# AntonXue/nn-sdp

Measured on NVIDIA B200. Metric: queries/sec (clique LMI blocks assembled: value * cliques_per_query), higher is better.
Workload: dtype f64

## Files before the change

include/nnsdp_b200.h:

```cpp
#ifndef NNSDP_B200_H
#define NNSDP_B200_H

#include <stdint.h>

#ifdef __cplusplus
extern "C" {
#endif

#define NNSDP_OK 0
#define NNSDP_ERR_ARG (-1)
#define NNSDP_ERR_CUDA (-2)
#define NNSDP_ERR_NOMEM (-3)
#define NNSDP_ERR_STATE (-4)
#define NNSDP_ERR_ASSERT (-5)
#define NNSDP_ERR_NOCONV (-6)

#define NNSDP_OUT_SAFETY 0
#define NNSDP_OUT_HPLANE 1
#define NNSDP_OUT_CIRCLE 2
#define NNSDP_OUT_ELLIPSOID 3

#define NNSDP_FORMAT_BLOCKS 0
#define NNSDP_FORMAT_DENSE_Z 1
#define NNSDP_FORMAT_PACKED 2
// ... 60 lines not shown
int32_t nnsdp_cliques(const nnsdp_net* net, int64_t beta, int64_t* ck_off, int64_t* ck_idx,
                      int64_t* ck1_len, int64_t* d_off, int64_t* d_idx);
int32_t nnsdp_sizes_from_xdims(int64_t K, const int64_t* xdims, int64_t beta, nnsdp_sizes* sizes);
int32_t nnsdp_cliques_from_xdims(int64_t K, const int64_t* xdims, int64_t beta, int64_t* ck_off,
                                 int64_t* ck_idx, int64_t* ck1_len, int64_t* d_off, int64_t* d_idx);

int32_t nnsdp_plan_stats(int64_t K, const int64_t* xdims, int64_t beta, int32_t dense_Z,
                         int64_t* tiles_per_prog, int64_t* entries_per_prog, int64_t* tile_rows,
                         int64_t* tile_cols);

int32_t nnsdp_plan_tiles(int64_t K, const int64_t* xdims, int64_t beta, int32_t dense_Z,
                         int64_t max_tiles, int32_t* tiles_out, int64_t* ntiles);

int32_t nnsdp_plan_panel(int64_t K, const int64_t* xdims, int64_t beta, int32_t dense_Z, int64_t max_items,
                         int64_t* items_out, int64_t* nitems);

int32_t nnsdp_gather_plan(int64_t K, const int64_t* xdims, int64_t beta, int32_t dense_Z, int64_t max_cells,
                          int32_t* cells_out, int64_t* ncells, int64_t max_thin, int64_t* thin_out,
                          int64_t* nthin, int32_t* usable);

int32_t nnsdp_bounds_ibp(nnsdp_ctx* ctx, const nnsdp_net* net, int64_t Q, const double* x1min,
                         const double* x1max, double* xmin, double* xmax, double* acxmin,
                         double* acxmax);
int32_t nnsdp_bounds_crown(nnsdp_ctx* ctx, const nnsdp_net* net, int64_t Q, const double* x1min,
                           const double* x1max, double* xmin, double* xmax, double* acxmin, double* acxmax);
int32_t nnsdp_preact_from_x(nnsdp_ctx* ctx, const nnsdp_net* net, int64_t Q, const double* xmin,
                            const double* xmax, double* acxmin, double* acxmax);
int32_t nnsdp_sector_minmax(nnsdp_ctx* ctx, int64_t n, const double* acxmin, const double* acxmax,
                            double* smin, double* smax);
int32_t nnsdp_assemble_blocks(nnsdp_ctx* ctx, const nnsdp_net* net, int64_t beta, int64_t Q,
// ... 110 lines not shown
```

nn-sdp_b200/csrc/api.cu:

```cuda
#include <math.h>
#include <stdarg.h>
#include <stdio.h>
#include <stdlib.h>
#include <string.h>

#include <algorithm>
#include <cmath>
#include <condition_variable>
#include <deque>
#include <functional>
#include <memory>
#include <mutex>
#include <thread>
#include <unordered_map>

#include <cuda.h>

#include "internal.h"

namespace nnsdp {

static thread_local std::string g_err;

void set_error(const char* fmt, ...) {
// ... 207 lines not shown
  DevBuf xmin, xmax, acxmin, acxmax, smin_c, smax_c;
  DevBuf d11, Md, T0, Bt, u, aff, part, act, cnt, Z11, Z1K, U;
  DevBuf gram, ringbuf, flags;
  DevBuf cr_rowsA, cr_rowsB, cr_bias, cr_prel, cr_preu, cr_du, cr_bu, cr_dl;
  DevBuf cr_keep_l, cr_keep_u;
  bool keep_preact = false, preact_valid = false;
  BatchDev bd{};
  GramDev gd{};
  PlanDev pd{};
  bool have_inputs = false, bounds_supplied = false, bounds_done = false, prepared = false;
  bool shared_gram = false;
  int bounds_method = 0;
  cudaStream_t st = nullptr, st_copy = nullptr;
  cudaEvent_t ev_start = nullptr, ev_stop = nullptr;
  cudaEvent_t ev_done[2] = {nullptr, nullptr}, ev_free[2] = {nullptr, nullptr};
  std::vector<StageSpan> spans;
  std::vector<cudaEvent_t> ev_pool;
  float stage_ms[ST_COUNT] = {};
  int64_t stage_launches[ST_COUNT] = {};

  cudaEvent_t get_event() {
    if (!ev_pool.empty()) {
      cudaEvent_t e = ev_pool.back();
      ev_pool.pop_back();
      return e;
    }
    cudaEvent_t e = nullptr;
    cudaEventCreate(&e);
    return e;
  }
// ... 15 lines not shown
    for (auto& sp : spans) {
      float ms = 0.f;
      if (cudaEventElapsedTime(&ms, sp.e0, sp.e1) == cudaSuccess) {
        stage_ms[sp.stage] += ms;
        if (sp.stage >= 5 && sp.stage <= 7) stage_ms[3] += ms;
      }
      ev_pool.push_back(sp.e0);
      ev_pool.push_back(sp.e1);
    }
    spans.clear();
  }
  std::vector<DevBuf*> all_bufs() {
    return {&d_bands, &d_tmaps, &d_tmap_ok, &d_tiles, &d_strips, &d_bulk, &d_mats, &d_panel, &d_goff, &d_ldG, &d_chol, &ze_netv, &ze_g, &ze_rows, &ze_part, &ze_io, &ze_err, &x1min, &x1max, &ymin, &ymax, &smin, &smax,
            &gin, &gbnd, &gsec, &outS, &outvec, &outinvP, &gout, &xmin, &xmax, &acxmin, &acxmax,
            &smin_c, &smax_c, &d11, &Md, &T0, &Bt, &u, &aff, &part, &act, &cnt, &Z11, &Z1K, &U,
            &gram, &ringbuf, &flags, &cr_rowsA, &cr_rowsB, &cr_bias, &cr_prel, &cr_preu, &cr_du, &cr_bu, &cr_dl,
            &cr_keep_l, &cr_keep_u};
  }
};

namespace {

int32_t require_device() {
  int n = 0;
  cudaError_t e = cudaGetDeviceCount(&n);
  if (e != cudaSuccess || n <= 0) {
    cudaGetLastError();
    set_error("no CUDA device available (%s); this library has no CPU fallback",
              e == cudaSuccess ? "device count is 0" : cudaGetErrorString(e));
    return NNSDP_ERR_CUDA;
  }
// ... 325 lines not shown
  Shape sh;
  NN_TRY(shape_from_xdims(K, xdims, &sh));
  nnsdp_sizes sz;
  NN_TRY(fill_sizes(sh, beta, &sz));
  std::vector<CliqueRanges> mats;
  NN_TRY(format_mats(sh, beta, dense_Z, &mats));
  PlanHost plan;
  PackedLayout lay;
  NN_TRY(build_plan(sh, beta, mats, true, &plan, dense_Z == NNSDP_FORMAT_PACKED ? &lay : nullptr));
  *ntiles = (int64_t)plan.tiles.size();
  if (tiles_out) {
    NN_CHECK(max_tiles >= *ntiles, NNSDP_ERR_ARG, "tiles_out too small");
    static_assert(sizeof(TileDev) == 11 * sizeof(int32_t), "TileDev layout");
    memcpy(tiles_out, plan.tiles.data(), plan.tiles.size() * sizeof(TileDev));
  }
  return NNSDP_OK;
}

int32_t nnsdp_plan_panel(int64_t K, const int64_t* xdims, int64_t beta, int32_t dense_Z, int64_t max_items,
                         int64_t* items_out, int64_t* nitems) {
  NN_CHECK(nitems != nullptr, NNSDP_ERR_ARG, "NULL argument");
  Shape sh;
  NN_TRY(shape_from_xdims(K, xdims, &sh));
  nnsdp_sizes sz;
  NN_TRY(fill_sizes(sh, beta, &sz));
  std::vector<CliqueRanges> mats;
  NN_TRY(format_mats(sh, beta, dense_Z, &mats));
  PlanHost plan;
  PackedLayout lay;
  NN_TRY(build_plan(sh, beta, mats, true, &plan, dense_Z == NNSDP_FORMAT_PACKED ? &lay : nullptr));
// ... 40 lines not shown
        o[5] = c.kind; o[6] = c.blk; o[7] = c.pure_zero;
      }
  }
  if (thin_out) {
    NN_CHECK(max_thin >= *nthin, NNSDP_ERR_ARG, "thin_out too small");
    memcpy(thin_out, gp.thin_idx.data(), gp.thin_idx.size() * 8);
  }
  return NNSDP_OK;
}

int32_t nnsdp_batch_destroy(nnsdp_batch* b) {
  if (!b) return NNSDP_OK;
  cudaSetDevice(b->dev);
  if (b->st) cudaStreamSynchronize(b->st);
  if (b->st_copy) cudaStreamSynchronize(b->st_copy);
  b->resolve_spans();
  b->pool.reset();
  for (DevBuf* x : b->all_bufs()) x->release();
  b->d_thin_idx.release();
  b->d_packed.release();
  b->d_pairs.release();
  if (b->h_packed) cudaFreeHost(b->h_packed);
  for (cudaEvent_t e : b->ev_packed)
    if (e) cudaEventDestroy(e);
  for (cudaEvent_t e : b->ev_pool) cudaEventDestroy(e);
  for (cudaEvent_t e : {b->ev_start, b->ev_stop, b->ev_done[0], b->ev_done[1], b->ev_free[0], b->ev_free[1]})
    if (e) cudaEventDestroy(e);
  if (b->st) cudaStreamDestroy(b->st);
  if (b->st_copy) cudaStreamDestroy(b->st_copy);
  delete b;
  return NNSDP_OK;
}

int32_t nnsdp_batch_create(nnsdp_ctx* ctx, int32_t dev_index, const nnsdp_net* net, int64_t beta,
                           int64_t Qcap, int64_t ring_queries, int32_t dense_Z, nnsdp_batch** out) {
  NN_CHECK(out != nullptr, NNSDP_ERR_ARG, "batch output pointer is NULL");
  *out = nullptr;
  NN_CHECK(ctx && net, NNSDP_ERR_ARG, "NULL argument");
  NN_CHECK(net->ctx == ctx, NNSDP_ERR_ARG, "net was uploaded through a different ctx");
  NN_CHECK(dev_index >= 0 && dev_index < (int)ctx->devs.size(), NNSDP_ERR_ARG, "bad dev_index");
  NN_CHECK(Qcap >= 1 && Qcap < (1 << 30), NNSDP_ERR_ARG, "bad Qcap");
  NN_CHECK(ring_queries >= 0 && ring_queries <= 65535, NNSDP_ERR_ARG, "ring_queries must be in [0, 65535]");
  const Shape& sh = net->sh;
  nnsdp_batch* b = new nnsdp_batch();
// ... 64 lines not shown
    for (const BandDev& j : b->plan.bands) b->band_max_m = std::max(b->band_max_m, j.m);
    b->nbands = (int)b->plan.bands.size();
    NN_TRY(upload(b->d_bands, b->plan.bands.data(), b->plan.bands.size() * sizeof(BandDev), b->st));
    if (!b->packed) NN_TRY(build_gather_plan(sh, beta, mats, b->plan, &b->gp));
    if (const char* e = getenv("NNSDP_DENSE_GATHER"))
      if (e[0] == '1') b->gp.usable = false;
    if (b->gp.usable) {
      NN_TRY(upload(b->d_thin_idx, b->gp.thin_idx.data(), b->gp.thin_idx.size() * 8, b->st));
      for (int i = 0; i < GATHER_STAGES; ++i)
        NN_CUDA(cudaEventCreateWithFlags(&b->ev_packed[i], cudaEventDisableTiming));
    }
    NN_TRY(upload(b->d_tiles, b->plan.tiles.data(), b->plan.tiles.size() * sizeof(TileDev), b->st));
    NN_TRY(upload(b->d_mats, b->plan.mats.data(), b->plan.mats.size() * sizeof(MatDev), b->st));
    NN_TRY(b->ringbuf.ensure((size_t)b->plan.per_query_doubles * b->ring * 8));
    b->slot_bulk.assign((size_t)b->ring * sh.K, 0);
    auto is_bulk = [&](const StripDev& d) {
      return !b->packed && d.rblk >= 1 && d.rblk <= sh.K - 1 &&
             (d.prog == PROG_SAME || (d.prog == PROG_DIAG && !b->plan.band_inline));
    };
    std::vector<StripDev> strips, bulk;
    std::vector<std::vector<StripDev>> per_blk(sh.K);
    b->pass_entries = 0;
    b->bulk_entries.assign(sh.K, 0);
    for (const StripDev& d : b->plan.strips) {
      if (d.prog == PROG_ZERO) continue;
      if (is_bulk(d)) {
        per_blk[d.rblk].push_back(d);
        b->bulk_entries[d.rblk] += (int64_t)d.nrows * d.ncols;
      } else {
        strips.push_back(d);
        b->pass_entries += (int64_t)d.nrows * d.ncols;
      }
    }
    b->bulk_begin.assign(sh.K + 1, 0);
// ... 4 lines not shown
    b->bulk_begin[sh.K] = (int)bulk.size();
    for (int i = b->plan.n_fill; i < (int)b->plan.tiles.size(); ++i)
      b->pass_entries += (int64_t)b->plan.tiles[i].nrows * b->plan.tiles[i].ncols;
    for (const BandDev& j : b->plan.bands)
      if (j.ld > 0) b->pass_entries += (int64_t)j.m * (2 * beta + 1) - beta * (beta + 1);
    NN_TRY(upload(b->d_strips, strips.data(), strips.size() * sizeof(StripDev), b->st));
    NN_TRY(upload(b->d_bulk, bulk.data(), bulk.size() * sizeof(StripDev), b->st));
    b->pd.strips = b->d_strips.as<StripDev>();
    b->pd.bulk = b->d_bulk.as<StripDev>();
    b->pd.n_strips = (int)strips.size();
    b->pd.tiles = b->d_tiles.as<TileDev>();
    b->pd.mats = b->d_mats.as<MatDev>();
    b->pd.panel_desc = nullptr;
    b->pd.n_panel = 0;
    b->pd.fold = 0;
    {
      static const int panel_env = [] { const char* e = getenv("NNSDP_PANEL"); return e ? atoi(e) : 1; }();
      if (panel_env && !b->packed && !b->plan.panel.empty()) {
        const char* fold_env = getenv("NNSDP_PANEL_FOLD");
        const bool fold = !(fold_env && atoi(fold_env) == 0);
        std::vector<StripDev> panel;
        for (const StripDev& d : fold ? b->plan.panel_fold : b->plan.panel)
          if (d.prog != PROG_ZERO && (d.prog == PROG_RC || d.prog == PROG_CR || !is_bulk(d))) panel.push_back(d);
        NN_TRY(upload(b->d_panel, panel.data(), panel.size() * sizeof(StripDev), b->st));
        b->pd.panel_desc = b->d_panel.as<StripDev>();
        b->pd.n_panel = (int)panel.size();
        b->pd.fold = fold ? 1 : 0;
      }
    }
    b->pd.ntiles = (int)b->plan.tiles.size();
    b->pd.n_fill = b->plan.n_fill;
    b->pd.n_window = b->plan.n_window;
    b->pd.n_edge = b->plan.n_edge;
    b->pd.tile_rows = b->plan.tile_rows;
    b->pd.per_query = b->plan.per_query_doubles;
    b->pd.tmaps = nullptr;
// ... 29 lines not shown
          NN_CUDA(cudaStreamSynchronize(b->st));
          b->pd.tmaps = b->d_tmaps.p;
          b->pd.tmap_ok = b->d_tmap_ok.as<int>();
        }
      } else {
        cudaGetLastError();
      }
    }
    b->pd.packed = b->plan.skip_absent ? 1 : 0;
    b->pd.band_inline = b->plan.band_inline ? 1 : 0;
    b->gd.scratch = b->gram.as<double>();
    b->gd.per_query = go;
    b->gd.goff = b->d_goff.as<long long>();
    b->gd.ldG = b->d_ldG.as<int>();
    b->gd.mirror = b->packed && b->plan.skip_absent ? 0 : 1;
  }
  NN_CUDA(cudaStreamSynchronize(b->st));
  guard.b = nullptr;
  *out = b;
  return NNSDP_OK;
}

int32_t nnsdp_batch_set_inputs(nnsdp_batch* b, int64_t Q, const nnsdp_query_inputs* in) {
  NN_CHECK(b && in, NNSDP_ERR_ARG, "NULL argument");
  NN_CHECK(Q >= 1 && Q <= b->Qcap, NNSDP_ERR_ARG, "Q = %lld outside [1, Qcap = %lld]", (long long)Q,
           (long long)b->Qcap);
  NN_CUDA(cudaSetDevice(b->dev));
  const Shape& sh = b->net->sh;
  const nnsdp_sizes& sz = b->sz;
  BatchDev& bd = b->bd;
// ... 215 lines not shown
    for (int blk = 1; blk < K; ++blk) {
      const int first = b->bulk_begin[blk], count = b->bulk_begin[blk + 1] - first;
      if (count == 0) continue;
      const bool now = blk <= K - 2 ? b->h_cnt[(size_t)q * K + blk] > 0 : b->bd.has_s22 != 0;
      if (now || held[blk]) {
        b->sel.push_back({(int32_t)i, first, count});
        entries += b->bulk_entries[blk];
      }
      held[blk] = now;
    }
  }
  if (!b->packed) b->emitted_bytes += entries * 8;
  return NNSDP_OK;
}

static int32_t emit_pass(nnsdp_batch* b, const GramDev& gd, int q0, int nq, double* dst) {
  const NetPerDev& nd = *b->nd;
  NN_TRY(prepare_slots(b, q0, nq, (dst - b->ringbuf.as<double>()) / b->plan.per_query_doubles));
  int total = 0;
  for (int which = 0; which < 3; ++which) {
    b->span_begin(ST_EMIT_FILL + which, b->st);
    const int l = launch_emit(nd.nd, b->bd, gd, b->pd, q0, nq, dst, b->st, which, b->sel.data(), (int)b->sel.size());
    b->span_end(b->st, l);
    total += l;
  }
  if (b->nbands > 0) {
    b->span_begin(ST_EMIT_EDGE, b->st);
    const int l = launch_emit_band(nd.nd, b->bd, gd, b->d_bands.as<BandDev>(), b->nbands, b->band_max_m, b->pd.per_query,
                                   q0, nq, dst, b->st);
    b->span_end(b->st, l);
    total += l;
  }
  b->stage_launches[ST_EMIT] += total;
  const cudaError_t e = cudaGetLastError();
  if (e != cudaSuccess) {
    b->ring_zeroed = 0;
    return cuda_fail(e, "emitter pass", __FILE__, __LINE__);
  }
  return NNSDP_OK;
}

int32_t nnsdp_batch_emit(nnsdp_batch* b, int64_t q0, int64_t nq) {
  NN_CHECK(b != nullptr, NNSDP_ERR_ARG, "batch is NULL");
  NN_CHECK(b->prepared, NNSDP_ERR_STATE, "nnsdp_batch_emit before nnsdp_batch_prepare");
  NN_CHECK(q0 >= 0 && nq >= 1 && q0 + nq <= b->Q && nq <= b->ring, NNSDP_ERR_ARG,
           "bad query range [%lld, %lld) for Q = %lld, ring = %lld", (long long)q0,
           (long long)(q0 + nq), (long long)b->Q, (long long)b->ring);
// ... 169 lines not shown
    const size_t need = (size_t)GATHER_STAGES * chunk * b->gp.thin_idx.size();
    if (need > b->h_packed_doubles) {
      if (b->h_packed) cudaFreeHost(b->h_packed);
      b->h_packed = nullptr;
      b->h_packed_doubles = 0;
      NN_CUDA(cudaHostAlloc((void**)&b->h_packed, std::max<size_t>(need, 1) * 8, cudaHostAllocPortable));
      b->h_packed_doubles = need;
      NN_TRY(b->d_packed.ensure(std::max<size_t>(need, 1) * 8));
    }
    if (!b->pool) {
      int nt = (int)std::min<unsigned>(16u, std::max(1u, std::thread::hardware_concurrency()));
      if (const char* e = getenv("NNSDP_HOST_THREADS")) nt = std::max(1, atoi(e));
      b->pool.reset(new WorkerPool(nt));
    }
  }
  bool used[2] = {false, false};
  int h = 0, ci = 0;
  int32_t status = NNSDP_OK;
  for (int64_t q0 = 0; q0 < b->Q && status == NNSDP_OK; q0 += chunk, h = (h + 1) % nhalf, ++ci) {
    const int64_t nq = std::min(chunk, b->Q - q0);
    double* dst = b->ringbuf.as<double>() + (int64_t)h * chunk * per;
    GramDev gd = b->gd;
    if (b->shared_gram) gd.per_query = 0;
    else gd.scratch += (int64_t)h * chunk * gd.per_query;
    if (sparse && ci >= GATHER_STAGES) b->pool->wait_group(ci - GATHER_STAGES);
    if (host_out && used[h]) NN_CUDA(cudaStreamWaitEvent(b->st, b->ev_free[h], 0));
    if (!b->shared_gram || ci == 0) {
      b->span_begin(ST_GRAM, b->st);
      int l = b->shared_gram
                  ? launch_gram(nd.nd, b->bd, b->gd, (int)b->net->max_block, 0, b->d_pairs.as<int>(), (int)b->pair_begin[1], b->st)
                  : launch_gram(nd.nd, b->bd, gd, (int)b->net->max_block, (int)q0, b->d_pairs.as<int>() + 2 * b->pair_begin[q0],
                                (int)(b->pair_begin[q0 + nq] - b->pair_begin[q0]), b->st);
      b->span_end(b->st, l > 0 ? l : 0);
      NN_CHECK(l >= 0, NNSDP_ERR_ARG, "a hidden layer of %lld neurons is too wide for the Gram kernel's grid",
               (long long)b->net->max_block);
      NN_CUDA(cudaGetLastError());
    }
    status = emit_pass(b, gd, (int)q0, (int)nq, dst);
    if (status != NNSDP_OK) break;
    if (sparse) {
      status = gather_chunk(b, ci, q0, nq, h, dst, host_out, flags);
      used[h] = true;
    } else if (host_out && b->packed && !(flags & NNSDP_RUN_DENSE_COPY)) {
      NN_CUDA(cudaEventRecord(b->ev_done[h], b->st));
      NN_CUDA(cudaStreamWaitEvent(b->st_copy, b->ev_done[h], 0));
      b->span_begin(ST_D2H, b->st_copy);
      const int64_t alw = b->lay.always_doubles;
      if (alw == per)
        NN_CUDA(cudaMemcpyAsync(host_out + q0 * per, dst, (size_t)nq * per * 8, cudaMemcpyDeviceToHost, b->st_copy));
      else
        NN_CUDA(cudaMemcpy2DAsync(host_out + q0 * per, (size_t)per * 8, dst, (size_t)per * 8, (size_t)alw * 8, (size_t)nq,
                                  cudaMemcpyDeviceToHost, b->st_copy));
      b->gather_bytes_dma += nq * alw * 8;
      for (int64_t q = q0; q < q0 + nq; ++q)
// ... 10 lines not shown
      used[h] = true;
    } else if (host_out) {
      NN_CUDA(cudaEventRecord(b->ev_done[h], b->st));
      NN_CUDA(cudaStreamWaitEvent(b->st_copy, b->ev_done[h], 0));
      b->span_begin(ST_D2H, b->st_copy);
      NN_CUDA(cudaMemcpyAsync(host_out + q0 * per, dst, (size_t)nq * per * 8, cudaMemcpyDeviceToHost,
                              b->st_copy));
      b->span_end(b->st_copy, 0);
      NN_CUDA(cudaEventRecord(b->ev_free[h], b->st_copy));
      used[h] = true;
      b->gather_bytes_dma += nq * per * 8;
    }
  }
  if (b->pool) b->pool->wait_all();
  if (status != NNSDP_OK) {
    cudaStreamSynchronize(b->st);
    cudaStreamSynchronize(b->st_copy);
    return status;
  }
  NN_CUDA(cudaGetLastError());
  NN_CUDA(cudaStreamSynchronize(b->st));
  NN_CUDA(cudaStreamSynchronize(b->st_copy));
  b->resolve_spans();
  return NNSDP_OK;
}

int32_t nnsdp_batch_run_ex(nnsdp_batch* b, double* host_out, int32_t flags) { return run_impl(b, host_out, nullptr, flags); }

int32_t nnsdp_batch_run(nnsdp_batch* b, double* host_out) { return run_impl(b, host_out, nullptr, 0); }

int32_t nnsdp_batch_run_packed(nnsdp_batch* b, double* host_records, uint8_t* present, int32_t flags) {
  NN_CHECK(b != nullptr, NNSDP_ERR_ARG, "batch is NULL");
  NN_CHECK(b->packed, NNSDP_ERR_STATE, "the batch was not created with NNSDP_FORMAT_PACKED");
// ... 1523 lines not shown
```

nn-sdp_b200/csrc/internal.h:

```cpp
#pragma once

#include <cuda_runtime.h>
#include <stdint.h>

#include <string>
#include <vector>

#include "../../include/nnsdp_b200.h"

namespace nnsdp {

void set_error(const char* fmt, ...);
int32_t cuda_fail(cudaError_t e, const char* what, const char* file, int line);

#define NN_CUDA(call)                                                                \
  do {                                                                               \
    cudaError_t _e = (call);                                                         \
    if (_e != cudaSuccess) return ::nnsdp::cuda_fail(_e, #call, __FILE__, __LINE__); \
  } while (0)

#define NN_CHECK(cond, code, ...)      \
  do {                                 \
    if (!(cond)) {                     \
      ::nnsdp::set_error(__VA_ARGS__); \
// ... 136 lines not shown
struct GatherColSeg {
  int32_t mat, col0, ncols;
  std::vector<GatherCell> cells;
};
struct GatherPlan {
  bool usable = false;
  std::vector<GatherColSeg> colsegs;
  std::vector<int32_t> colseg_begin;
  std::vector<int64_t> thin_idx;
  std::vector<int64_t> thin_begin;
  int64_t dense_always_doubles = 0;
};

int32_t build_plan(const Shape& sh, int64_t beta, const std::vector<CliqueRanges>& mats,
                   bool classify, PlanHost* plan, PackedLayout* packed = nullptr);
void unpack_record(const Shape& sh, int64_t beta, const PackedLayout& lay, const std::vector<CliqueRanges>& mats,
                   const double* record, const uint8_t* present, double* out);
int32_t build_gather_plan(const Shape& sh, int64_t beta, const std::vector<CliqueRanges>& mats,
                          const PlanHost& plan, GatherPlan* gp);

struct CholFront {
  long long out_off;
  long long g0;
  int n, npriv;
  int lead, tail;
};
int32_t build_chol_plan(const Shape& sh, const std::vector<CliqueRanges>& mats, std::vector<CholFront>* fronts);

struct NetDev {
  int K, n_in, n_out, Zdim, acdim, xtot;
// ... 204 lines not shown
```

nn-sdp_b200/csrc/kernels_emit.cu:

```cuda
#include <stdlib.h>

#include <algorithm>

#include "internal.h"

namespace nnsdp {

namespace {

constexpr int ETHREADS = 256;
constexpr int SLOT_GROUP = 8;
constexpr int FAST_TR = 128, FAST_TC = 32, FAST_NCOL = 16;
constexpr int MAX_TAPS = 2 * MAX_FAST_BETA + 1;
constexpr int MAX_TC = 32;

struct QView {
  const double* Md;
  const double* T0;
  const double* Bt;
  const double* gbnd;
  const double* aff;
  const double* Z11;
  const double* Z1K;
  const double* U;
// ... 726 lines not shown
    const dim3 grid(plan.n_window * ((nq + wgroup - 1) / wgroup));
    const int t0 = plan.n_fill;
    static const int gm_env = [] { const char* e = getenv("NNSDP_WINDOW_GROUP_MAJOR"); return e ? atoi(e) : -1; }();
    const int gm = gm_env >= 0 ? gm_env : plan.band_inline;
    switch (b.beta) {
      case 0: emit_window_kernel<0><<<grid, ETHREADS, 0, st>>>(net, b, plan, t0, q0, nq, wgroup, gm, out); break;
      case 1: emit_window_kernel<1><<<grid, ETHREADS, 0, st>>>(net, b, plan, t0, q0, nq, wgroup, gm, out); break;
      case 2: emit_window_kernel<2><<<grid, ETHREADS, 0, st>>>(net, b, plan, t0, q0, nq, wgroup, gm, out); break;
      case 3: emit_window_kernel<3><<<grid, ETHREADS, 0, st>>>(net, b, plan, t0, q0, nq, wgroup, gm, out); break;
      case 4: emit_window_kernel<4><<<grid, ETHREADS, 0, st>>>(net, b, plan, t0, q0, nq, wgroup, gm, out); break;
      default: return -1;
    }
    ++launches;
  }
  }
  if (which < 0 || which == 0) launches += launch_bulk(net, b, g, plan, q0, sel, nsel, out, st);
  if (!plan.fold && plan.n_edge > 0 && (which < 0 || which == 2)) {
    emit_edge_kernel<<<dim3(plan.n_edge, (nq + egroup - 1) / egroup), ETHREADS, 0, st>>>(
        net, b, g, plan, plan.n_fill + plan.n_window, q0, nq, egroup, out);
    ++launches;
  }
  return launches;
}

}
```

nn-sdp_b200/csrc/plan.cpp:

```cpp
#include <stdint.h>
#include <stdlib.h>

#include <algorithm>

#include "internal.h"
#include <atomic>
#include <cstring>
#include <thread>

namespace nnsdp {

int64_t lambda_dim(int64_t acdim, int64_t beta) {
  int64_t s = 0;
  for (int64_t t = acdim - beta; t <= acdim; ++t) s += t;
  return s;
}

long long gram_layout(const Shape& sh, std::vector<long long>* goff, std::vector<int>* ldG) {
  goff->assign(sh.K, 0);
  ldG->assign(sh.K, 0);
  long long go = 0;
  for (int blk = 0; blk <= sh.K - 2; ++blk) {
    (*ldG)[blk] = (int)(((sh.n[blk] + 15) / 16) * 16);
    (*goff)[blk] = go;
    go += (long long)(*ldG)[blk] * sh.n[blk];
  }
  return go;
}

static int64_t Sfun(const Shape& sh, int64_t k) {
// ... 848 lines not shown
```

nn-sdp_b200/nnsdp_b200/__init__.py:

```python
from . import _lib
from ._lib import NnsdpError, device_count, OUT_SAFETY, OUT_HPLANE, OUT_CIRCLE, OUT_ELLIPSOID, RUN_HOST_PREZEROED, RUN_DENSE_COPY, FORMAT_BLOCKS, FORMAT_DENSE_Z, FORMAT_PACKED, CELL_WINDOW, CELL_DIAG, CELL_BAND, CELL_RECT
from .core import (Context, Net, Batch, NumericBatch, PinnedBuffer, assemble_blocks, assemble_dense,
                   bounds_ibp, bounds_crown, preact_from_x, sector_minmax, split_blocks, sizes_from_xdims,
                   cliques_from_xdims, plan_stats, plan_tiles, plan_panel, certify_plan, assembly_error_nmax, affine_form, affine_form_batch, gather_plan, read_nnet, read_vnnlib, packed_layout, packed_unpack,
                   assemble_packed)
from . import reference_api
```

nn-sdp_b200/nnsdp_b200/_lib.py:

```python
from __future__ import annotations

import ctypes as C
import os

_HERE = os.path.dirname(os.path.abspath(__file__))
LIB_PATH = os.environ.get("NNSDP_B200_LIB", os.path.join(_HERE, "..", "lib", "libnnsdp_b200.so"))

OK, ERR_ARG, ERR_CUDA, ERR_NOMEM, ERR_STATE, ERR_ASSERT, ERR_NOCONV = 0, -1, -2, -3, -4, -5, -6
OUT_SAFETY, OUT_HPLANE, OUT_CIRCLE, OUT_ELLIPSOID = 0, 1, 2, 3
RUN_HOST_PREZEROED, RUN_DENSE_COPY = 1, 2
FORMAT_BLOCKS, FORMAT_DENSE_Z, FORMAT_PACKED = 0, 1, 2
CELL_WINDOW, CELL_DIAG, CELL_BAND, CELL_RECT = 1, 2, 3, 4

c_i32, c_i64, c_u64 = C.c_int32, C.c_int64, C.c_uint64
c_dp = C.POINTER(C.c_double)
c_i64p = C.POINTER(C.c_int64)
c_vp = C.c_void_p


class Sizes(C.Structure):
    _fields_ = [(n, c_i64) for n in (
        "K", "Zdim", "acdim", "xtot", "lamdim", "secdim", "n_in", "n_out", "sdim", "ncliques",
        "sum_ck", "sum_ck_sq", "sum_dk", "max_ck")]

# ... 48 lines not shown
    "nnsdp_ctx_destroy": (c_i32, [c_vp]),
    "nnsdp_ctx_num_devices": (c_i32, [c_vp, C.POINTER(c_i32)]),
    "nnsdp_host_alloc": (c_i32, [c_u64, C.POINTER(c_vp)]),
    "nnsdp_host_free": (c_i32, [c_vp]),
    "nnsdp_net_upload": (c_i32, [c_vp, c_i64, c_i64p, C.POINTER(c_dp), C.POINTER(c_vp)]),
    "nnsdp_net_destroy": (c_i32, [c_vp]),
    "nnsdp_nnet_read": (c_i32, [C.c_char_p, c_i64, c_i64p, c_i64p, c_i64, c_dp, c_i64p]),
    "nnsdp_vnnlib_read": (c_i32, [C.c_char_p, c_i64, c_i64, c_i64, c_i64p, c_i64p, c_dp, c_dp, c_dp, c_i64p]),
    "nnsdp_query_sizes": (c_i32, [c_vp, c_i64, C.POINTER(Sizes)]),
    "nnsdp_cliques": (c_i32, [c_vp, c_i64, c_i64p, c_i64p, c_i64p, c_i64p, c_i64p]),
    "nnsdp_sizes_from_xdims": (c_i32, [c_i64, c_i64p, c_i64, C.POINTER(Sizes)]),
    "nnsdp_cliques_from_xdims": (c_i32, [c_i64, c_i64p, c_i64, c_i64p, c_i64p, c_i64p, c_i64p, c_i64p]),
    "nnsdp_plan_stats": (c_i32, [c_i64, c_i64p, c_i64, c_i32, c_i64p, c_i64p, c_i64p, c_i64p]),
    "nnsdp_plan_tiles": (c_i32, [c_i64, c_i64p, c_i64, c_i32, c_i64, C.POINTER(c_i32), c_i64p]),
    "nnsdp_plan_panel": (c_i32, [c_i64, c_i64p, c_i64, c_i32, c_i64, c_i64p, c_i64p]),
    "nnsdp_gather_plan": (c_i32, [c_i64, c_i64p, c_i64, c_i32, c_i64, C.POINTER(c_i32), c_i64p, c_i64, c_i64p, c_i64p, C.POINTER(c_i32)]),
    "nnsdp_bounds_ibp": (c_i32, [c_vp, c_vp, c_i64, c_dp, c_dp, c_dp, c_dp, c_dp, c_dp]),
    "nnsdp_bounds_crown": (c_i32, [c_vp, c_vp, c_i64, c_dp, c_dp, c_dp, c_dp, c_dp, c_dp]),
    "nnsdp_batch_bounds_crown": (c_i32, [c_vp]),
    "nnsdp_batch_set_bounds_method": (c_i32, [c_vp, c_i32]),
    "nnsdp_batch_keep_crown_preact": (c_i32, [c_vp, c_i32]),
    "nnsdp_batch_get_crown_preact": (c_i32, [c_vp, c_dp, c_dp]),
    "nnsdp_preact_from_x": (c_i32, [c_vp, c_vp, c_i64, c_dp, c_dp, c_dp, c_dp]),
    "nnsdp_sector_minmax": (c_i32, [c_vp, c_i64, c_dp, c_dp, c_dp, c_dp]),
    "nnsdp_assemble_blocks": (c_i32, [c_vp, c_vp, c_i64, c_i64, C.POINTER(QueryInputs), c_dp]),
    "nnsdp_assemble_dense": (c_i32, [c_vp, c_vp, c_i64, c_i64, C.POINTER(QueryInputs), c_dp]),
    "nnsdp_batch_lambda_max": (c_i32, [c_vp, c_i32, C.c_double, c_dp, C.POINTER(c_i32)]),
    "nnsdp_batch_lambda_max_ex": (c_i32, [c_vp, c_i32, C.c_double, c_dp, C.POINTER(c_i32), c_dp, C.POINTER(c_i32)]),
    "nnsdp_batch_certify": (c_i32, [c_vp, c_dp, c_i64, C.POINTER(c_i32), c_dp, c_i64p, c_dp]),
    "nnsdp_batch_certify_ex": (c_i32, [c_vp, c_dp, c_i64, C.POINTER(c_i32), c_dp, c_i64p, c_dp, c_dp]),
# ... 75 lines not shown
```

nn-sdp_b200/nnsdp_b200/core.py:

```python
from __future__ import annotations

import ctypes as C
from dataclasses import dataclass
from typing import List, Optional, Sequence

import numpy as np

from . import _lib as L

STAGES = {"bounds": 0, "prepare": 1, "gram": 2, "emit": 3, "d2h": 4, "emit_fill": 5, "emit_window": 6, "emit_edge": 7}


def _dp(a: Optional[np.ndarray]):
    return None if a is None else a.ctypes.data_as(L.c_dp)


def _f64(a, shape_tail=None) -> np.ndarray:
    a = np.ascontiguousarray(np.asarray(a, dtype=np.float64))
    return a


class Context:

    def __init__(self, devices=None):
# ... 118 lines not shown
TILE_FIELDS = ("mat", "row0", "nrows", "col0", "ncols", "grow0", "gcol0", "flags", "rblk", "cblk", "prog")


PANEL_FIELDS = ("out_off", "ld", "row0", "nrows", "col0", "ncols", "grow0", "gcol0", "prog", "rblk")


def plan_panel(xdims: Sequence[int], beta: int, dense: int = 0) -> np.ndarray:
    K = len(xdims) - 1
    xd = (L.c_i64 * (K + 1))(*[int(x) for x in xdims])
    n = L.c_i64(0)
    L.check(L.lib.nnsdp_plan_panel(K, xd, beta, int(dense), 0, None, C.byref(n)))
    out = np.zeros((int(n.value), 10), dtype=np.int64)
    if n.value:
        L.check(L.lib.nnsdp_plan_panel(K, xd, beta, int(dense), int(n.value), out.ctypes.data_as(L.c_i64p), C.byref(n)))
    return out


CERTIFY_PLAN_FIELDS = ("out_off", "n", "npriv", "g0", "lead", "tail")


def assembly_error_nmax(xdims: Sequence[int], beta: int, out_kind: int) -> int:
    xd = np.ascontiguousarray(xdims, dtype=np.int64)
    n = L.c_i64(0)
    L.check(L.lib.nnsdp_assembly_error_nmax(len(xd) - 1, xd.ctypes.data_as(L.c_i64p), beta, out_kind, C.byref(n)))
    return int(n.value)


def certify_plan(xdims: Sequence[int], beta: int) -> np.ndarray:
    K = len(xdims) - 1
    xd = (L.c_i64 * (K + 1))(*[int(x) for x in xdims])
# ... 515 lines not shown
```

Measured before the change: 9468.

## Overlap next-chunk Gram and band emission on a side stream

Adds a high-priority side stream that computes the Gram scratch for the next chunk while the current chunk is emitted, using a second Gram buffer and events to ping-pong between them. When a plan-time check shows that band writers do not overlap the other emit writers, the band-edge kernel also runs on the side stream, concurrently with the fill kernels. This is meant to hide Gram and band kernel latency behind the emit work. The cost is extra memory for the second buffer, more event synchronisation, and correctness that depends on the disjointness check.

```diff
diff --git a/include/nnsdp_b200.h b/include/nnsdp_b200.h
--- a/include/nnsdp_b200.h
+++ b/include/nnsdp_b200.h
@@ -98,6 +98,9 @@
 
 int32_t nnsdp_plan_panel(int64_t K, const int64_t* xdims, int64_t beta, int32_t dense_Z, int64_t max_items,
                          int64_t* items_out, int64_t* nitems);
+
+int32_t nnsdp_plan_band_disjoint(int64_t K, const int64_t* xdims, int64_t beta, int32_t dense_Z, const int64_t* items,
+                                 int64_t nitems, int32_t* disjoint);
 
 int32_t nnsdp_gather_plan(int64_t K, const int64_t* xdims, int64_t beta, int32_t dense_Z, int64_t max_cells,
                           int32_t* cells_out, int64_t* ncells, int64_t max_thin, int64_t* thin_out,
diff --git a/nn-sdp_b200/csrc/api.cu b/nn-sdp_b200/csrc/api.cu
--- a/nn-sdp_b200/csrc/api.cu
+++ b/nn-sdp_b200/csrc/api.cu
@@ -245,6 +245,11 @@
   cudaStream_t st = nullptr, st_copy = nullptr;
   cudaEvent_t ev_start = nullptr, ev_stop = nullptr;
   cudaEvent_t ev_done[2] = {nullptr, nullptr}, ev_free[2] = {nullptr, nullptr};
+  bool overlap = false, band_beside = false;
+  cudaStream_t st_side = nullptr;
+  cudaEvent_t ev_gram[2] = {nullptr, nullptr}, ev_fill[2] = {nullptr, nullptr}, ev_band[2] = {nullptr, nullptr};
+  cudaEvent_t ev_join = nullptr;
+  DevBuf gram2;
   std::vector<StageSpan> spans;
   std::vector<cudaEvent_t> ev_pool;
   float stage_ms[ST_COUNT] = {};
@@ -290,7 +295,7 @@
     return {&d_bands, &d_tmaps, &d_tmap_ok, &d_tiles, &d_strips, &d_bulk, &d_mats, &d_panel, &d_goff, &d_ldG, &d_chol, &ze_netv, &ze_g, &ze_rows, &ze_part, &ze_io, &ze_err, &x1min, &x1max, &ymin, &ymax, &smin, &smax,
             &gin, &gbnd, &gsec, &outS, &outvec, &outinvP, &gout, &xmin, &xmax, &acxmin, &acxmax,
             &smin_c, &smax_c, &d11, &Md, &T0, &Bt, &u, &aff, &part, &act, &cnt, &Z11, &Z1K, &U,
-            &gram, &ringbuf, &flags, &cr_rowsA, &cr_rowsB, &cr_bias, &cr_prel, &cr_preu, &cr_du, &cr_bu, &cr_dl,
+            &gram, &gram2, &ringbuf, &flags, &cr_rowsA, &cr_rowsB, &cr_bias, &cr_prel, &cr_preu, &cr_du, &cr_bu, &cr_dl,
             &cr_keep_l, &cr_keep_u};
   }
 };
@@ -646,6 +651,39 @@
     static_assert(sizeof(TileDev) == 11 * sizeof(int32_t), "TileDev layout");
     memcpy(tiles_out, plan.tiles.data(), plan.tiles.size() * sizeof(TileDev));
   }
+  return NNSDP_OK;
+}
+
+static bool is_bulk_strip(const StripDev& d, int K, const PlanHost& plan, bool packed) {
+  return !packed && d.rblk >= 1 && d.rblk <= K - 1 && (d.prog == PROG_SAME || (d.prog == PROG_DIAG && !plan.band_inline));
+}
+
+int32_t nnsdp_plan_band_disjoint(int64_t K, const int64_t* xdims, int64_t beta, int32_t dense_Z, const int64_t* items,
+                                 int64_t nitems, int32_t* disjoint) {
+  NN_CHECK(disjoint != nullptr && (items != nullptr || nitems == 0) && nitems >= 0, NNSDP_ERR_ARG, "bad argument");
+  Shape sh;
+  NN_TRY(shape_from_xdims(K, xdims, &sh));
+  nnsdp_sizes sz;
+  NN_TRY(fill_sizes(sh, beta, &sz));
+  std::vector<CliqueRanges> mats;
+  NN_TRY(format_mats(sh, beta, dense_Z, &mats));
+  PlanHost plan;
+  PackedLayout lay;
+  const bool packed = dense_Z == NNSDP_FORMAT_PACKED;
+  NN_TRY(build_plan(sh, beta, mats, true, &plan, packed ? &lay : nullptr));
+  std::vector<StripDev> w;
+  for (const StripDev& d : plan.strips)
+    if (d.prog != PROG_ZERO && !is_bulk_strip(d, sh.K, plan, packed)) w.push_back(d);
+  for (const StripDev& d : plan.panel_fold)
+    if (d.prog != PROG_ZERO && !is_bulk_strip(d, sh.K, plan, packed)) w.push_back(d);
+  for (int64_t i = 0; i < nitems; ++i) {
+    const int64_t* it = items + 6 * i;
+    StripDev d{};
+    d.out_off = it[0];
+    d.ld = (int32_t)it[1], d.row0 = (int32_t)it[2], d.nrows = (int32_t)it[3], d.col0 = (int32_t)it[4], d.ncols = (int32_t)it[5];
+    w.push_back(d);
+  }
+  *disjoint = band_writers_disjoint(w, plan.bands, beta) ? 1 : 0;
   return NNSDP_OK;
 }
 
@@ -716,6 +754,7 @@
   cudaSetDevice(b->dev);
   if (b->st) cudaStreamSynchronize(b->st);
   if (b->st_copy) cudaStreamSynchronize(b->st_copy);
+  if (b->st_side) cudaStreamSynchronize(b->st_side);
   b->resolve_spans();
   b->pool.reset();
   for (DevBuf* x : b->all_bufs()) x->release();
@@ -726,10 +765,12 @@
   for (cudaEvent_t e : b->ev_packed)
     if (e) cudaEventDestroy(e);
   for (cudaEvent_t e : b->ev_pool) cudaEventDestroy(e);
-  for (cudaEvent_t e : {b->ev_start, b->ev_stop, b->ev_done[0], b->ev_done[1], b->ev_free[0], b->ev_free[1]})
+  for (cudaEvent_t e : {b->ev_start, b->ev_stop, b->ev_done[0], b->ev_done[1], b->ev_free[0], b->ev_free[1], b->ev_gram[0],
+                        b->ev_gram[1], b->ev_fill[0], b->ev_fill[1], b->ev_band[0], b->ev_band[1], b->ev_join})
     if (e) cudaEventDestroy(e);
   if (b->st) cudaStreamDestroy(b->st);
   if (b->st_copy) cudaStreamDestroy(b->st_copy);
+  if (b->st_side) cudaStreamDestroy(b->st_side);
   delete b;
   return NNSDP_OK;
 }
@@ -824,10 +865,7 @@
     NN_TRY(upload(b->d_mats, b->plan.mats.data(), b->plan.mats.size() * sizeof(MatDev), b->st));
     NN_TRY(b->ringbuf.ensure((size_t)b->plan.per_query_doubles * b->ring * 8));
     b->slot_bulk.assign((size_t)b->ring * sh.K, 0);
-    auto is_bulk = [&](const StripDev& d) {
-      return !b->packed && d.rblk >= 1 && d.rblk <= sh.K - 1 &&
-             (d.prog == PROG_SAME || (d.prog == PROG_DIAG && !b->plan.band_inline));
-    };
+    auto is_bulk = [&](const StripDev& d) { return is_bulk_strip(d, sh.K, b->plan, b->packed); };
     std::vector<StripDev> strips, bulk;
     std::vector<std::vector<StripDev>> per_blk(sh.K);
     b->pass_entries = 0;
@@ -862,12 +900,12 @@
     b->pd.panel_desc = nullptr;
     b->pd.n_panel = 0;
     b->pd.fold = 0;
+    std::vector<StripDev> panel;
     {
       static const int panel_env = [] { const char* e = getenv("NNSDP_PANEL"); return e ? atoi(e) : 1; }();
       if (panel_env && !b->packed && !b->plan.panel.empty()) {
         const char* fold_env = getenv("NNSDP_PANEL_FOLD");
         const bool fold = !(fold_env && atoi(fold_env) == 0);
-        std::vector<StripDev> panel;
         for (const StripDev& d : fold ? b->plan.panel_fold : b->plan.panel)
           if (d.prog != PROG_ZERO && (d.prog == PROG_RC || d.prog == PROG_CR || !is_bulk(d))) panel.push_back(d);
         NN_TRY(upload(b->d_panel, panel.data(), panel.size() * sizeof(StripDev), b->st));
@@ -927,6 +965,19 @@
     b->gd.goff = b->d_goff.as<long long>();
     b->gd.ldG = b->d_ldG.as<int>();
     b->gd.mirror = b->packed && b->plan.skip_absent ? 0 : 1;
+    const char* ov_env = getenv("NNSDP_OVERLAP");
+    b->overlap = !b->packed && !(ov_env && atoi(ov_env) == 0);
+    if (b->overlap) {
+      int least = 0, greatest = 0;
+      NN_CUDA(cudaDeviceGetStreamPriorityRange(&least, &greatest));
+      const char* pe = getenv("NNSDP_OVERLAP_PRIO");
+      NN_CUDA(cudaStreamCreateWithPriority(&b->st_side, cudaStreamNonBlocking, (pe && atoi(pe) == 0) ? least : greatest));
+      for (cudaEvent_t* e : {&b->ev_gram[0], &b->ev_gram[1], &b->ev_fill[0], &b->ev_fill[1], &b->ev_band[0],
+                             &b->ev_band[1], &b->ev_join})
+        NN_CUDA(cudaEventCreateWithFlags(e, cudaEventDisableTiming));
+      if (b->ring >= 2) NN_TRY(b->gram2.ensure((size_t)go * b->ring * 8));
+      b->band_beside = atoi(ov_env ? ov_env : "1") != 2 && b->nbands > 0 && band_writers_disjoint(b->pd.n_panel > 0 && beta <= MAX_WINDOW_BETA ? panel : strips, b->plan.bands, beta);
+    }
   }
   NN_CUDA(cudaStreamSynchronize(b->st));
   guard.b = nullptr;
@@ -1172,23 +1223,35 @@
   return NNSDP_OK;
 }
 
-static int32_t emit_pass(nnsdp_batch* b, const GramDev& gd, int q0, int nq, double* dst) {
+static int32_t emit_pass(nnsdp_batch* b, const GramDev& gd, int q0, int nq, double* dst, int pass = -1) {
   const NetPerDev& nd = *b->nd;
+  const bool band_side = pass >= 0 && b->band_beside;
   NN_TRY(prepare_slots(b, q0, nq, (dst - b->ringbuf.as<double>()) / b->plan.per_query_doubles));
   int total = 0;
   for (int which = 0; which < 3; ++which) {
     b->span_begin(ST_EMIT_FILL + which, b->st);
-    const int l = launch_emit(nd.nd, b->bd, gd, b->pd, q0, nq, dst, b->st, which, b->sel.data(), (int)b->sel.size());
+    int l = launch_emit(nd.nd, b->bd, gd, b->pd, q0, nq, dst, b->st, which, nullptr, 0);
+    if (which == 0) {
+      if (band_side && pass > 0) NN_CUDA(cudaStreamWaitEvent(b->st, b->ev_band[(pass - 1) & 1], 0));
+      l += launch_emit(nd.nd, b->bd, gd, b->pd, q0, nq, dst, b->st, 3, b->sel.data(), (int)b->sel.size());
+    }
     b->span_end(b->st, l);
     total += l;
   }
+  if (band_side) {
+    NN_CUDA(cudaEventRecord(b->ev_fill[pass & 1], b->st));
+    NN_CUDA(cudaStreamWaitEvent(b->st_side, b->ev_fill[pass & 1], 0));
+  }
   if (b->nbands > 0) {
-    b->span_begin(ST_EMIT_EDGE, b->st);
+    cudaStream_t s = band_side ? b->st_side : b->st;
+    b->span_begin(ST_EMIT_EDGE, s);
     const int l = launch_emit_band(nd.nd, b->bd, gd, b->d_bands.as<BandDev>(), b->nbands, b->band_max_m, b->pd.per_query,
-                                   q0, nq, dst, b->st);
-    b->span_end(b->st, l);
+                                   q0, nq, dst, s);
+    b->span_end(s, l);
     total += l;
   }
+  if (band_side) NN_CUDA(cudaEventRecord(b->ev_band[pass & 1], b->st_side));
+  else if (pass >= 0) NN_CUDA(cudaEventRecord(b->ev_fill[pass & 1], b->st));
   b->stage_launches[ST_EMIT] += total;
   const cudaError_t e = cudaGetLastError();
   if (e != cudaSuccess) {
@@ -1388,30 +1451,56 @@
       b->pool.reset(new WorkerPool(nt));
     }
   }
+  const bool gram_side = b->overlap && !(getenv("NNSDP_OVERLAP") && atoi(getenv("NNSDP_OVERLAP")) == 3) && !b->shared_gram && (nhalf == 2 || b->gram2.p != nullptr);
+  const bool side = gram_side || (b->overlap && b->band_beside);
+  auto gram_of = [&](int pass) {
+    GramDev gd = b->gd;
+    if (b->shared_gram) gd.per_query = 0;
+    else if (nhalf == 2) gd.scratch += (int64_t)(pass % 2) * chunk * gd.per_query;
+    else if (gram_side && pass % 2 == 1) gd.scratch = b->gram2.as<double>();
+    return gd;
+  };
+  auto gram_pass = [&](int pass, cudaStream_t s) -> int32_t {
+    const int64_t q0 = pass * chunk, nq = std::min(chunk, b->Q - q0);
+    b->span_begin(ST_GRAM, s);
+    int l = b->shared_gram
+                ? launch_gram(nd.nd, b->bd, b->gd, (int)b->net->max_block, 0, b->d_pairs.as<int>(), (int)b->pair_begin[1], s)
+                : launch_gram(nd.nd, b->bd, gram_of(pass), (int)b->net->max_block, (int)q0,
+                              b->d_pairs.as<int>() + 2 * b->pair_begin[q0], (int)(b->pair_begin[q0 + nq] - b->pair_begin[q0]), s);
+    b->span_end(s, l > 0 ? l : 0);
+    NN_CHECK(l >= 0, NNSDP_ERR_ARG, "a hidden layer of %lld neurons is too wide for the Gram kernel's grid",
+             (long long)b->net->max_block);
+    NN_CUDA(cudaGetLastError());
+    return NNSDP_OK;
+  };
   bool used[2] = {false, false};
   int h = 0, ci = 0;
   int32_t status = NNSDP_OK;
+  if (side) {
+    NN_CUDA(cudaEventRecord(b->ev_join, b->st));
+    NN_CUDA(cudaStreamWaitEvent(b->st_side, b->ev_join, 0));
+  }
   for (int64_t q0 = 0; q0 < b->Q && status == NNSDP_OK; q0 += chunk, h = (h + 1) % nhalf, ++ci) {
     const int64_t nq = std::min(chunk, b->Q - q0);
     double* dst = b->ringbuf.as<double>() + (int64_t)h * chunk * per;
-    GramDev gd = b->gd;
-    if (b->shared_gram) gd.per_query = 0;
-    else gd.scratch += (int64_t)h * chunk * gd.per_query;
+    const GramDev gd = gram_of(ci);
     if (sparse && ci >= GATHER_STAGES) b->pool->wait_group(ci - GATHER_STAGES);
     if (host_out && used[h]) NN_CUDA(cudaStreamWaitEvent(b->st, b->ev_free[h], 0));
-    if (!b->shared_gram || ci == 0) {
-      b->span_begin(ST_GRAM, b->st);
-      int l = b->shared_gram
-                  ? launch_gram(nd.nd, b->bd, b->gd, (int)b->net->max_block, 0, b->d_pairs.as<int>(), (int)b->pair_begin[1], b->st)
-                  : launch_gram(nd.nd, b->bd, gd, (int)b->net->max_block, (int)q0, b->d_pairs.as<int>() + 2 * b->pair_begin[q0],
-                                (int)(b->pair_begin[q0 + nq] - b->pair_begin[q0]), b->st);
-      b->span_end(b->st, l > 0 ? l : 0);
-      NN_CHECK(l >= 0, NNSDP_ERR_ARG, "a hidden layer of %lld neurons is too wide for the Gram kernel's grid",
-               (long long)b->net->max_block);
-      NN_CUDA(cudaGetLastError());
-    }
-    status = emit_pass(b, gd, (int)q0, (int)nq, dst);
+    if (gram_side) {
+      if (ci == 0) status = gram_pass(0, b->st);
+      else NN_CUDA(cudaStreamWaitEvent(b->st, b->ev_gram[ci & 1], 0));
+      if (status == NNSDP_OK && q0 + chunk < b->Q) {
+        if (ci > 0) NN_CUDA(cudaStreamWaitEvent(b->st_side, b->ev_fill[(ci - 1) & 1], 0));
+        status = gram_pass(ci + 1, b->st_side);
+        NN_CUDA(cudaEventRecord(b->ev_gram[(ci + 1) & 1], b->st_side));
+      }
+    } else if (!b->shared_gram || ci == 0) {
+      status = gram_pass(ci, b->st);
+    }
     if (status != NNSDP_OK) break;
+    status = emit_pass(b, gd, (int)q0, (int)nq, dst, side ? ci : -1);
+    if (status != NNSDP_OK) break;
+    if (host_out && side && b->band_beside) NN_CUDA(cudaStreamWaitEvent(b->st, b->ev_band[ci & 1], 0));
     if (sparse) {
       status = gather_chunk(b, ci, q0, nq, h, dst, host_out, flags);
       used[h] = true;
@@ -1452,9 +1541,14 @@
   }
   if (b->pool) b->pool->wait_all();
   if (status != NNSDP_OK) {
+    if (side) cudaStreamSynchronize(b->st_side);
     cudaStreamSynchronize(b->st);
     cudaStreamSynchronize(b->st_copy);
     return status;
+  }
+  if (side) {
+    NN_CUDA(cudaEventRecord(b->ev_join, b->st_side));
+    NN_CUDA(cudaStreamWaitEvent(b->st, b->ev_join, 0));
   }
   NN_CUDA(cudaGetLastError());
   NN_CUDA(cudaStreamSynchronize(b->st));
diff --git a/nn-sdp_b200/csrc/internal.h b/nn-sdp_b200/csrc/internal.h
--- a/nn-sdp_b200/csrc/internal.h
+++ b/nn-sdp_b200/csrc/internal.h
@@ -174,6 +174,7 @@
 
 int32_t build_plan(const Shape& sh, int64_t beta, const std::vector<CliqueRanges>& mats,
                    bool classify, PlanHost* plan, PackedLayout* packed = nullptr);
+bool band_writers_disjoint(const std::vector<StripDev>& items, const std::vector<BandDev>& bands, int64_t beta);
 void unpack_record(const Shape& sh, int64_t beta, const PackedLayout& lay, const std::vector<CliqueRanges>& mats,
                    const double* record, const uint8_t* present, double* out);
 int32_t build_gather_plan(const Shape& sh, int64_t beta, const std::vector<CliqueRanges>& mats,
diff --git a/nn-sdp_b200/csrc/kernels_emit.cu b/nn-sdp_b200/csrc/kernels_emit.cu
--- a/nn-sdp_b200/csrc/kernels_emit.cu
+++ b/nn-sdp_b200/csrc/kernels_emit.cu
@@ -764,7 +764,7 @@
     ++launches;
   }
   }
-  if (which < 0 || which == 0) launches += launch_bulk(net, b, g, plan, q0, sel, nsel, out, st);
+  if (which < 0 || which == 0 || which == 3) launches += launch_bulk(net, b, g, plan, q0, sel, nsel, out, st);
   if (!plan.fold && plan.n_edge > 0 && (which < 0 || which == 2)) {
     emit_edge_kernel<<<dim3(plan.n_edge, (nq + egroup - 1) / egroup), ETHREADS, 0, st>>>(
         net, b, g, plan, plan.n_fill + plan.n_window, q0, nq, egroup, out);
diff --git a/nn-sdp_b200/csrc/plan.cpp b/nn-sdp_b200/csrc/plan.cpp
--- a/nn-sdp_b200/csrc/plan.cpp
+++ b/nn-sdp_b200/csrc/plan.cpp
@@ -14,6 +14,24 @@
   int64_t s = 0;
   for (int64_t t = acdim - beta; t <= acdim; ++t) s += t;
   return s;
+}
+
+bool band_writers_disjoint(const std::vector<StripDev>& items, const std::vector<BandDev>& bands, int64_t beta) {
+  for (const BandDev& bd : bands) {
+    if (bd.band_off >= 0 || bd.optional || bd.upper_only) return false;
+    if (bd.ld <= 0) continue;
+    for (const StripDev& d : items) {
+      if (d.out_off != bd.out_off) continue;
+      if (d.ld != bd.ld) return false;
+      for (int64_t t = -beta; t <= beta; ++t) {
+        const int64_t lo = std::max({(int64_t)0, -t, (int64_t)d.row0 - bd.row0, (int64_t)d.col0 - bd.col0 - t});
+        const int64_t hi = std::min({(int64_t)bd.m, bd.m - t, (int64_t)d.row0 + d.nrows - bd.row0,
+                                     (int64_t)d.col0 + d.ncols - bd.col0 - t});
+        if (lo < hi) return false;
+      }
+    }
+  }
+  return true;
 }
 
 long long gram_layout(const Shape& sh, std::vector<long long>* goff, std::vector<int>* ldG) {
diff --git a/nn-sdp_b200/nnsdp_b200/__init__.py b/nn-sdp_b200/nnsdp_b200/__init__.py
--- a/nn-sdp_b200/nnsdp_b200/__init__.py
+++ b/nn-sdp_b200/nnsdp_b200/__init__.py
@@ -2,6 +2,6 @@
 from ._lib import NnsdpError, device_count, OUT_SAFETY, OUT_HPLANE, OUT_CIRCLE, OUT_ELLIPSOID, RUN_HOST_PREZEROED, RUN_DENSE_COPY, FORMAT_BLOCKS, FORMAT_DENSE_Z, FORMAT_PACKED, CELL_WINDOW, CELL_DIAG, CELL_BAND, CELL_RECT
 from .core import (Context, Net, Batch, NumericBatch, PinnedBuffer, assemble_blocks, assemble_dense,
                    bounds_ibp, bounds_crown, preact_from_x, sector_minmax, split_blocks, sizes_from_xdims,
-                   cliques_from_xdims, plan_stats, plan_tiles, plan_panel, certify_plan, assembly_error_nmax, affine_form, affine_form_batch, gather_plan, read_nnet, read_vnnlib, packed_layout, packed_unpack,
+                   cliques_from_xdims, plan_stats, plan_tiles, plan_panel, plan_band_disjoint, certify_plan, assembly_error_nmax, affine_form, affine_form_batch, gather_plan, read_nnet, read_vnnlib, packed_layout, packed_unpack,
                    assemble_packed)
 from . import reference_api
diff --git a/nn-sdp_b200/nnsdp_b200/_lib.py b/nn-sdp_b200/nnsdp_b200/_lib.py
--- a/nn-sdp_b200/nnsdp_b200/_lib.py
+++ b/nn-sdp_b200/nnsdp_b200/_lib.py
@@ -86,6 +86,7 @@
     "nnsdp_plan_stats": (c_i32, [c_i64, c_i64p, c_i64, c_i32, c_i64p, c_i64p, c_i64p, c_i64p]),
     "nnsdp_plan_tiles": (c_i32, [c_i64, c_i64p, c_i64, c_i32, c_i64, C.POINTER(c_i32), c_i64p]),
     "nnsdp_plan_panel": (c_i32, [c_i64, c_i64p, c_i64, c_i32, c_i64, c_i64p, c_i64p]),
+    "nnsdp_plan_band_disjoint": (c_i32, [c_i64, c_i64p, c_i64, c_i32, c_i64p, c_i64, C.POINTER(c_i32)]),
     "nnsdp_gather_plan": (c_i32, [c_i64, c_i64p, c_i64, c_i32, c_i64, C.POINTER(c_i32), c_i64p, c_i64, c_i64p, c_i64p, C.POINTER(c_i32)]),
     "nnsdp_bounds_ibp": (c_i32, [c_vp, c_vp, c_i64, c_dp, c_dp, c_dp, c_dp, c_dp, c_dp]),
     "nnsdp_bounds_crown": (c_i32, [c_vp, c_vp, c_i64, c_dp, c_dp, c_dp, c_dp, c_dp, c_dp]),
diff --git a/nn-sdp_b200/nnsdp_b200/core.py b/nn-sdp_b200/nnsdp_b200/core.py
--- a/nn-sdp_b200/nnsdp_b200/core.py
+++ b/nn-sdp_b200/nnsdp_b200/core.py
@@ -156,6 +156,15 @@
     if n.value:
         L.check(L.lib.nnsdp_plan_panel(K, xd, beta, int(dense), int(n.value), out.ctypes.data_as(L.c_i64p), C.byref(n)))
     return out
+
+
+def plan_band_disjoint(xdims: Sequence[int], beta: int, dense: int = 0, items=None) -> bool:
+    K = len(xdims) - 1
+    xd = (L.c_i64 * (K + 1))(*[int(x) for x in xdims])
+    it = np.ascontiguousarray(np.zeros((0, 6)) if items is None else items, dtype=np.int64).reshape(-1, 6)
+    ok = L.c_i32(0)
+    L.check(L.lib.nnsdp_plan_band_disjoint(K, xd, beta, int(dense), it.ctypes.data_as(L.c_i64p), len(it), C.byref(ok)))
+    return bool(ok.value)
 
 
 CERTIFY_PLAN_FIELDS = ("out_off", "n", "npriv", "g0", "lead", "tail")
```

Measured after the change: 9648 (median of 6 runs). +1.9%, better.
